# sleepybishop/nanorq

Measured on AMD Instinct MI355X. Metric: Gbit/s encode+decode, K=8192 T=1280, higher is better.
Workload: dtype u8

## Files before the change

__graft_entry__.py:

```python
import os
import sys

ROOT = os.path.dirname(os.path.abspath(__file__))
for p in (ROOT, os.path.join(ROOT, "tests")):
    if p not in sys.path:
        sys.path.insert(0, p)


def build():
    from nanorq_amd import build as nbuild
    nbuild.build_lib(verbose=True)
    nbuild.build_emu()
    nbuild.build_planner_emu()
    nbuild.build_ingest_emu()
    nbuild.build_emit_emu()
    nbuild.build_held_emu()
    nbuild.build_rxset_emu()
    nbuild.build_rxset_lists_emu()
    nbuild.build_txset_emu()
    nbuild.build_obj_emu()
    nbuild.build_shape_emu()
    nbuild.build_tools()
    import oracle
    oracle.build()
    if os.path.isfile("/root/reference/benchmark.c"):
        import subprocess
        subprocess.run(["make", "-s", "-C", os.path.join(ROOT, "oracle"), "_ref/benchmark_hip", "_ref/encode_hip", "_ref/decode_hip"],
                       check=True)
    import nanorq_amd
    nanorq_amd.lib()
    print("build ok:", nanorq_amd.lib_path())


def smoke():
    import numpy as np
# ... 29 lines not shown
```

nanorq_amd/binding.py:

```python
import ctypes as C
import os

import numpy as np

_HERE = os.path.dirname(os.path.abspath(__file__))
_LIB = None


class NrqError(RuntimeError):
    pass


class ObjParams(C.Structure):
    _fields_ = [("F", C.c_uint64)] + [(n, C.c_uint32) for n in
                                       ("T", "Al", "Z", "N", "Kt", "ZL", "KL", "KpL", "ZS", "KS", "KpS", "NL", "TL", "NS", "TS",
                                        "flags", "max_esi")] + [("oti_common", C.c_uint64), ("oti_specific", C.c_uint32)]

    def as_dict(self):
        return {n: getattr(self, n) for n, _ in self._fields_}


class CallStats(C.Structure):
    _fields_ = [("plan_ms", C.c_double), ("host_ms", C.c_double), ("strip_bytes", C.c_uint32),
                ("lds_bytes", C.c_uint32), ("grid", C.c_uint32), ("planner", C.c_uint32),
# ... 121 lines not shown
        L.nrq_rxset_decode.argtypes = [vp, ip, u32p]
    if hasattr(L, "nrq_txset_create"):
        L.nrq_txset_create.argtypes = [vp, C.c_uint32, C.POINTER(vp)]
        L.nrq_txset_destroy.argtypes = [vp]
        L.nrq_txset_destroy.restype = None
        L.nrq_txset_attach.argtypes = [vp, C.c_uint32, vp]
        L.nrq_txset_attach_obj.argtypes = [vp, C.c_uint32, vp]
        L.nrq_txset_detach.argtypes = [vp, C.c_uint32]
        L.nrq_txset_blocks.argtypes = [vp, u32p, u32p, C.c_uint32, u32p]
        L.nrq_txset_emit.argtypes = [vp, vp, vp, C.c_uint32, vp, sz, C.c_uint32, vp]
    u8pp = C.POINTER(C.POINTER(C.c_uint8))
    L.nrq_host_kconst_build.argtypes = [C.c_uint32, u8pp, u32p]
    L.nrq_host_plan_build.argtypes = [C.c_uint32, C.c_uint32, u32p, C.POINTER(C.c_uint8), u8pp, u32p]
    L.nrq_host_free.argtypes = [vp]
    L.nrq_host_free.restype = None
    _LIB = L
    return L


PARAM_NAMES = ("Kp", "J", "S", "H", "W", "L", "P", "P1", "U", "B")
PLAN_FIELDS = ("magic status K Kp J S H W L P P1 B M npiv u nlow r2 nfree nlev nrows pipe wpr "
               "npiv_pad n_xor_ops off_ops off_pivslot off_pivcol off_wt off_lowslot off_pivx off_fbits "
               "off_mh off_freex off_hinv off_colslot off_pivof off_uslot total_bytes reserved0 reserved1 fail_site "
               "off_augt lpr aug_stride nneed need_pad off_needslot off_wneed").split()


def params(K):
    out = (C.c_uint32 * 10)()
    if lib().nrq_params(K, out) != 0:
        raise ValueError("K out of range: %r" % (K,))
    return dict(zip(PARAM_NAMES, (int(x) for x in out)))


def _u32(a):
    return a.ctypes.data_as(C.POINTER(C.c_uint32))


def host_kconst(K):
    out = C.POINTER(C.c_uint8)()
    n = C.c_uint32()
    if lib().nrq_host_kconst_build(K, C.byref(out), C.byref(n)) != 0:
        raise NrqError("kconst build failed")
    buf = bytes(C.string_at(out, n.value))
    lib().nrq_host_free(out)
    return buf


# ... 664 lines not shown
```

nanorq_amd/build.py:

```python
import os
import shutil
import subprocess
import sys

HERE = os.path.dirname(os.path.abspath(__file__))
ROOT = os.path.dirname(HERE)
CSRC = os.path.join(HERE, "csrc")
LIB = os.path.join(HERE, "libnanorq_hip.so")
EMU = os.path.join(ROOT, "tests", "emu", "libsolve_emu.so")
PEMU = os.path.join(ROOT, "tests", "emu", "libplanner_emu.so")
IEMU = os.path.join(ROOT, "tests", "emu", "libingest_emu.so")
XEMU = os.path.join(ROOT, "tests", "emu", "libemit_emu.so")
OEMU = os.path.join(ROOT, "tests", "emu", "libobj_emu.so")
SEMU = os.path.join(ROOT, "tests", "emu", "libshape_emu.so")
HEMU = os.path.join(ROOT, "tests", "emu", "libheld_emu.so")
WEMU = os.path.join(ROOT, "tests", "emu", "libwant_emu.so")
REMU = os.path.join(ROOT, "tests", "emu", "librxset_emu.so")
LEMU = os.path.join(ROOT, "tests", "emu", "librxset_lists_emu.so")
TEMU = os.path.join(ROOT, "tests", "emu", "libtxset_emu.so")

HIP_SOURCES = ["nrq_device.hip"]
CXX_SOURCES = ["planner_host.cpp"]
C_SOURCES = ["nanorq_api.c", "io.c"]


def _hipcc():
    for c in (os.environ.get("HIPCC"), "/opt/rocm/bin/hipcc", shutil.which("hipcc")):
        if c and os.path.exists(c):
            return c
    raise RuntimeError("hipcc not found: the HIP extension cannot be built (no CPU fallback exists)")


def _newer(target, deps):
# ... 54 lines not shown
    return target


def build_tools(force=False):
    src = os.path.join(ROOT, "tools", "rqfile.c")
    exe = os.path.join(ROOT, "tools", "rqfile")
    deps = [src, LIB] + [os.path.join(ROOT, "include", h) for h in ("nanorq.h", "nanorq_batch.h", "io.h")]
    if force or _newer(exe, deps):
        subprocess.run(["gcc", "-std=c99", "-D_DEFAULT_SOURCE", "-D_FILE_OFFSET_BITS=64", "-O2", "-Wall", "-I" + os.path.join(ROOT, "include"),
                        src, "-o", exe, "-L" + os.path.dirname(LIB), "-lnanorq_hip", "-Wl,-rpath,$ORIGIN/../nanorq_amd", "-lm"], check=True)
    return exe


def _build_emu(target, src, headers, force):
    if force or _newer(target, [src] + [os.path.join(CSRC, h) for h in headers]):
        subprocess.run(["g++", "-O2", "-std=c++17", "-Wall", "-Wno-unknown-pragmas", "-fPIC", "-shared", "-o", target, src], check=True)
    return target


def build_emu(force=False):
    return _build_emu(EMU, os.path.join(ROOT, "tests", "emu", "solve_emu.cpp"), ("solve_body.h", "plan.h"), force)


def build_planner_emu(force=False):
    return _build_emu(PEMU, os.path.join(ROOT, "tests", "emu", "planner_emu.cpp"),
                      ("planner_body.h", "planner_seq.h", "solve_body.h", "plan.h", "rq_math.h"), force)


def build_ingest_emu(force=False):
    return _build_emu(IEMU, os.path.join(ROOT, "tests", "emu", "ingest_emu.cpp"), ("ingest_body.h",), force)


def build_emit_emu(force=False):
    return _build_emu(XEMU, os.path.join(CSRC, "emit_emu.cpp"), ("emit_body.h", "rq_math.h"), force)


def build_held_emu(force=False):
    return _build_emu(HEMU, os.path.join(CSRC, "held_emu.cpp"), ("emit_body.h", "held_body.h", "ingest_body.h", "rq_math.h"), force)


def build_want_emu(force=False):
    return _build_emu(WEMU, os.path.join(CSRC, "want_emu.cpp"), ("want_body.h", "held_body.h", "ingest_body.h"), force)


def build_rxset_emu(force=False):
    return _build_emu(REMU, os.path.join(CSRC, "rxset_emu.cpp"), ("ingest_set_body.h", "ingest_body.h"), force)


def build_rxset_lists_emu(force=False):
    return _build_emu(LEMU, os.path.join(CSRC, "rxset_lists_emu.cpp"),
                      ("lists_set_body.h", "rxset_plan.h", "ingest_set_body.h", "ingest_body.h"), force)


def build_txset_emu(force=False):
    return _build_emu(TEMU, os.path.join(CSRC, "txset_emu.cpp"), ("emit_set_body.h", "emit_body.h", "rq_math.h"), force)


def build_obj_emu(force=False):
    return _build_emu(OEMU, os.path.join(ROOT, "tests", "emu", "obj_emu.cpp"), ("obj_body.h", "emit_body.h", "rq_math.h"), force)


def build_shape_emu(force=False):
    return _build_emu(SEMU, os.path.join(ROOT, "tests", "emu", "shape_emu.cpp"),
                      ("launch_shape.h", "planner_body.h", "solve_body.h", "plan.h", "rq_math.h", "rfc6330_tables.h"), force)


if __name__ == "__main__":
    build_lib(force="-f" in sys.argv, verbose=True)
    build_emu(force="-f" in sys.argv)
    build_planner_emu(force="-f" in sys.argv)
    build_ingest_emu(force="-f" in sys.argv)
    build_emit_emu(force="-f" in sys.argv)
    build_held_emu(force="-f" in sys.argv)
    build_want_emu(force="-f" in sys.argv)
    build_rxset_emu(force="-f" in sys.argv)
    build_rxset_lists_emu(force="-f" in sys.argv)
    build_txset_emu(force="-f" in sys.argv)
    build_obj_emu(force="-f" in sys.argv)
    build_shape_emu(force="-f" in sys.argv)
    build_tools(force="-f" in sys.argv)
```

nanorq_amd/csrc/launch_shape.h:

```cpp
#ifndef NRQ_LAUNCH_SHAPE_H
#define NRQ_LAUNCH_SHAPE_H

#include <stdint.h>
#include <stdlib.h>
#include <string.h>

#include <vector>

#include "plan.h"
#include "rq_math.h"
#include "solve_body.h"
#include "planner_body.h"

#define NRQ_LDS_MAX 163840u
#define NRQ_LDS_GRANULE 1280u
static inline uint32_t lds_alloc(uint32_t bytes) { return (bytes + NRQ_LDS_GRANULE - 1u) / NRQ_LDS_GRANULE * NRQ_LDS_GRANULE; }
#ifndef NRQ_WG
#define NRQ_WG 768
#endif
#ifndef NRQ_TINY_WV
#define NRQ_TINY_WV 3
#endif
#ifndef NRQ_TINY_OCC
#define NRQ_TINY_OCC 12u
#endif
#ifndef NRQ_SMALL_WV
#define NRQ_SMALL_WV 4
#endif

static inline bool nrq_map_by_block(uint32_t nblk) { return nblk >= 64u || (nblk >= 8u && (nblk & 7u) == 0u); }

enum KnobKind { KNOB_FLAG, KNOB_NFLAG, KNOB_NUM, KNOB_BOOLNUM, KNOB_WIDEG, KNOB_LDSMAX };
#define NRQ_KNOBS(K)                                                                                                                                    \
  K(bool, map_spread, false, "NRQ_MAP_SPREAD", "map_spread", KNOB_FLAG)               \
  K(bool, big_wg, false, "NRQ_BIG_WG", "big_wg", KNOB_FLAG)                                                \
                                                                                                                          \
  K(bool, small_waves4, true, "NRQ_SMALL_WAVES5", "small_waves4", KNOB_NFLAG)                                                                           \
  K(bool, prof, false, "NRQ_PROF", 0, KNOB_FLAG)                                                   \
  K(bool, diag, false, "NRQ_DIAG", 0, KNOB_FLAG)                                                 \
  K(bool, plan_lds_max, false, "NRQ_PLAN_LDS_MAX", 0, KNOB_FLAG)                                                \
  K(bool, plan_big_wg, false, "NRQ_PLAN_BIG_WG", "plan_big_wg", KNOB_FLAG)                                             \
  K(uint32_t, small_div, 2, "NRQ_SMALL_DIV", 0, KNOB_NUM)        \
  K(uint64_t, solve_grid, 0, "NRQ_SOLVE_GRID", "solve_grid", KNOB_NUM)             \
  K(uint32_t, max_wb, 16, "NRQ_MAX_WB", "max_wb", KNOB_NUM)                                                                \
  K(bool, no_wb12, false, "NRQ_NO_WB12", "no_wb12", KNOB_FLAG)                                       \
                                                                                                    \
  K(bool, tiny_any, false, "NRQ_TINY_ANY", "tiny_any", KNOB_FLAG)                                                                                       \
  K(bool, plan_pack, false, "NRQ_PLAN_PACK", "plan_pack", KNOB_FLAG)          \
                                                              \
  K(bool, host_plan_auto, true, "NRQ_HOST_PLAN_AUTO", "host_plan_auto", KNOB_BOOLNUM)                                                                   \
  K(int, prof_base, 2, "NRQ_PROF_BASE", 0, KNOB_NUM)                                    \
                                                                                                        \
  K(uint32_t, encplan_dev_min_l, 12000, "NRQ_ENCPLAN_DEV_MIN_L", "encplan_dev_min_l", KNOB_NUM)                                                         \
  K(uint32_t, wide_g, 0, "NRQ_WIDE_G", "wide_g", KNOB_WIDEG)           \
                                                                  \
  K(bool, no_wentry, false, "NRQ_NO_WENTRY", "no_wentry", KNOB_FLAG)                                                                                    \
  K(bool, no_tiny, false, "NRQ_NO_TINY", "no_tiny", KNOB_FLAG)                                     \
                                                                                                            \
  K(uint32_t, tiny_div, 7, "NRQ_TINY_DIV", "tiny_div", KNOB_NUM)                                                                                        \
                                                                                                             \
  K(uint32_t, tiny_div_dec, 7, "NRQ_TINY_DIV_DEC", "tiny_div_dec", KNOB_NUM)                                                                            \
  K(bool, no_split, false, "NRQ_NO_SPLIT", "no_split", KNOB_FLAG)                \
  K(bool, no_balance, false, "NRQ_NO_BALANCE", "no_balance", KNOB_FLAG)            \
                                                    \
  K(uint32_t, lds_max, NRQ_LDS_MAX, 0, "lds_max", KNOB_LDSMAX)                                                                                          \
                                                                \
  K(bool, no_lists, false, "NRQ_NO_LISTS", "no_lists", KNOB_FLAG)                                                                                       \
  K(int, reserve_cus, -1, "NRQ_RESERVE_CUS", "reserve_cus", KNOB_NUM)  \
// ... 332 lines not shown
```

nanorq_amd/csrc/nrq_device.hip:

```cpp
#include <hip/hip_runtime.h>

#include <algorithm>
#include <atomic>
#include <chrono>
#include <cstdarg>
#include <cstdio>
#include <cstdlib>
#include <cstring>
#include <deque>
#include <map>
#include <new>
#include <string>
#include <thread>
#include <vector>

#include "../../include/nanorq_hip.h"
#include "plan.h"
#include "planner_host.h"
#include "rq_math.h"
#include "solve_body.h"
#include "planner_body.h"
#include "ingest_body.h"
#include "ingest_set_body.h"
#include "lists_set_body.h"
// ... 52 lines not shown
#endif
#ifndef NRQ_BIG_RING
#define NRQ_BIG_RING NRQ_RING_MAX
#endif
#ifndef NRQ_PROF_DONE
#define NRQ_PROF_DONE 9
#endif
#ifndef NRQ_W12_FW
#define NRQ_W12_FW 3
#endif
#ifndef NRQ_W12_GW
#define NRQ_W12_GW 2
#endif
#ifndef NRQ_W12_SW
#define NRQ_W12_SW 2
#endif
template <int WB, int NT, int WV, int G = 1, bool AL = false>
__global__ __launch_bounds__(NT) __attribute__((amdgpu_waves_per_eu(WV)))
void nrq_solve_kernel(const nrq_job *__restrict__ jobs, uint32_t nblk,
                                                       uint32_t T, uint32_t nstrips, uint32_t by_block, uint32_t nslots,
                                                       uint32_t lsub, const uint8_t *__restrict__ kc,
                                                       uint8_t *__restrict__ stage_all, uint32_t stage_stride,
                                                       uint32_t ostage_stride, unsigned long long *__restrict__ prof,
                                                       uint8_t *__restrict__ ybuf, size_t ybuf_stride) {
  extern __shared__ __attribute__((aligned(16))) uint8_t smem[];
  const uint32_t tid = threadIdx.x;
  static_assert(G == 1 || WB == 16, "wide strips are made of 16-byte lanes");
  static_assert(WB != 12 || NT >= 512, "12-byte strips: the 768-thread workgroup only (blocks whose 16-byte image does not fit the LDS)");
  constexpr uint32_t WBE = (uint32_t)WB * G;
  constexpr bool ALX = AL && G == 1 && WB >= 4;
  const uint32_t vt = tid / G, subl = tid % G;
  constexpr uint32_t VNT = NT / G;
  constexpr uint32_t SPL = nrq_group_strips(WBE), NFW = (G == 1 && WB == 12 && NT >= 512) ? (uint32_t)NRQ_W12_FW : (G == 1 && WB >= 8 && NT >= 512) ? 2u : 1u,
                     NMV = (NT / 64u) / 4u * (4u - NFW) + ((NT / 64u) % 4u > NFW ? (NT / 64u) % 4u - NFW : 0u),
                     NGW = NFW == 3u ? (uint32_t)NRQ_W12_GW : NMV >= 6u ? (WB <= NRQ_GATHER_WAVES_NARROW_WB ? NRQ_GATHER_WAVES_NARROW : NRQ_MOVER_WAVES) : NMV >= 3u ? 2u : 1u,
                     NSW = NFW == 3u ? (uint32_t)NRQ_W12_SW : NMV >= 6u ? NRQ_MOVER_WAVES : NMV - NGW;
  static_assert(NMV >= 2u || NT == 64, "workgroup too small for the data movers");
#ifndef NRQ_PIPE_SMALL
#define NRQ_PIPE_SMALL 0
#endif
#ifndef NRQ_PIPE_BIG
#define NRQ_PIPE_BIG 1
#endif
  constexpr bool MPIPE = (NRQ_PIPE_BIG && NT >= 512) || (NRQ_PIPE_SMALL && NT == 256 && WV == 4);
#ifndef NRQ_RING_4W
#define NRQ_RING_4W NRQ_RING
#endif
// ... 195 lines not shown
        ph_combine<WB, G>(c, w0, vt, VNT, cb_);
        __syncthreads();
      }
      if (lpr_) {
        ph_clear_x<WB, G>(c, vt, VNT);
        __syncthreads();
      }
      NRQ_STAMP(4);
      NRQ_STOP(3)
#ifndef NRQ_FOLD_PRE256
#define NRQ_FOLD_PRE256 0
#endif
      ph_dense_fold<WB, G, (NT == 64 ? 8 : NT == 256 ? NRQ_FOLD_PRE256 : 0)>(c, vt, VNT);
      __syncthreads();
      NRQ_MARK(c, 4);
      if (dense_fold_shared(VNT) || G > 1) {
        ph_hdpc_reduce<WB, G>(c, vt, VNT);
        __syncthreads();
      }
      NRQ_MARK(c, 5);
      ph_dense_free<WB, G, (NT == 64)>(c, vt, VNT);
      __syncthreads();
      NRQ_MARK(c, 6);
      ph_dense_cu<WB, G, (NT == 64)>(c, vt, VNT);
      __syncthreads();
      NRQ_STAMP(5);
      NRQ_STOP(4)
      if (ybuf) {
        NRQ_STAMP(6);
        NRQ_STAMP(7);
        ph_store_raw<WB, G>(c, ostage_cur + (size_t)sidx * ostage_stride + subl * WB, vt, VNT);
      } else {
        ph_tables<WB, G>(c, vt, VNT);
        __syncthreads();
        NRQ_STAMP(6);
        NRQ_STOP(5)
        ph_backsub<WB, G, (NT >= 512)>(c, vt, VNT);
        ph_park<WB, G>(c, vt, VNT);
        __syncthreads();
        NRQ_STAMP(7);
        NRQ_STOP(6)
        ph_store<WB, G, (NT >= 512)>(c, ostage_cur + (size_t)sidx * ostage_stride + subl * WB, vt, VNT);
      }
      __syncthreads();
      NRQ_STAMP(8);
#undef NRQ_STAMP
#undef NRQ_STOP
    }
    __syncthreads();
    qp = q;
    q = qn;
    buf ^= 1u;
  }
  if (qp < nslots) {
    GroupDst<WB> gp;
    const uint32_t units_p = group_dst(qp, gp) << lsub;
    pf_scatter_impl<WB, G, MPIPE, ALX>(gp, ostage0 + (size_t)(buf ^ 1u) * SPL * ostage_stride, ostage_stride, 0u, units_p, (tid) / G, (NT) / G, subl);
  }
}

enum {
// ... 880 lines not shown
    rc = 1;
    if (ctx->planner && p.L >= ctx->tune.encplan_dev_min_l) rc = encplan_device_launch(ctx, p, K, kc, ep);
    if (rc < 0) return rc;
    if (rc > 0) return encplan_host_build(ctx, p, K, kc, ep);
  }
  return finish ? encplan_finish(ctx, p, K, kc, ep) : 0;
}

void build_out_lists(const rq_params &p, const uint16_t *colslot, uint32_t n, const uint32_t *isis,
                     std::vector<uint32_t> &cptr, std::vector<uint16_t> &cols) {
  cptr.resize(n + 1);
  cols.clear();
  cols.reserve((size_t)n * 9);
  uint32_t tmp[RQ_MAX_LT_COLS];
  for (uint32_t q = 0; q < n; q++) {
    cptr[q] = (uint32_t)cols.size();
    uint32_t m = rq_lt_columns(&p, isis[q], tmp);
    for (uint32_t k = 0; k < m; k++) cols.push_back(colslot[tmp[k]]);
  }
  cptr[n] = (uint32_t)cols.size();
}

using solve_fn = void (*)(const nrq_job *, uint32_t, uint32_t, uint32_t, uint32_t, uint32_t, uint32_t, const uint8_t *, uint8_t *, uint32_t,
                          uint32_t, unsigned long long *, uint8_t *, size_t);
#define NRQ_SOLVE_ROW(WB, NT, WV, G, AL) &nrq_solve_kernel<WB, NT, WV, G, AL>,
static const solve_fn solve_table[] = {NRQ_SOLVE_INSTANCES(NRQ_SOLVE_ROW)};
#undef NRQ_SOLVE_ROW

static int launch_solve(nrq_ctx *ctx, const std::vector<const nrq_plan_hdr *> &hdrs, const nrq_job *d_jobs, uint32_t nblk,
                        uint32_t T, const uint8_t *d_kc, uint32_t max_out, uint32_t wb, uint32_t need, bool io_aligned) {
  SolveIn in;
  in.wb = wb; in.nblk = nblk; in.T = T; in.lds_bytes = need; in.max_out = max_out; in.io_aligned = io_aligned;
  in.hdrs = hdrs.data(); in.nhdrs = hdrs.size();
  for (const nrq_plan_hdr *h : hdrs) {
    if (h->status) continue;
    if (h->M > in.max_slots) in.max_slots = h->M;
    if (h->u > in.max_u) in.max_u = h->u;
    if (h->wpr > in.max_wpr) in.max_wpr = h->wpr;
  }
  const SolveShape s = solve_shape(ctx->tune, ctx->ncu, ctx->ahead_hint, in);
  if (s.err == SHAPE_GRID_TOO_LARGE) return fail(ctx, -4, "grid too large");
  if (s.key.NT == 64 && ctx->tune.diag) fprintf(stderr, "[NRQ_DIAG] single-wave workgroups: %u bytes of LDS each, %u per CU\n", s.lds_bytes, s.occ);
  const int inst = solve_key_index(s.key);
  if (inst < 0)
    return fail(ctx, -2, "no solve kernel instance <%d, %d, %d, %d, %s>", s.key.WB, s.key.NT, s.key.WV, s.key.G, s.key.AL ? "true" : "false");
  {
    int rc_ = ensure_dev(ctx, ctx->stage, s.stage_bytes());
// ... 10 lines not shown
                                    hipFuncAttributeMaxDynamicSharedMemorySize, (int)NRQ_LDS_MAX));
    HIPCHK(ctx, hipFuncSetAttribute(reinterpret_cast<const void *>(&nrq_backsub_kernel<16>),
                                    hipFuncAttributeMaxDynamicSharedMemorySize, (int)NRQ_LDS_MAX));
    for (int i = 0; i < nrq_solve_nkeys; i++)
      if (nrq_solve_keys[i].WB == (int)wb)
        HIPCHK(ctx, hipFuncSetAttribute(reinterpret_cast<const void *>(solve_table[i]), hipFuncAttributeMaxDynamicSharedMemorySize,
                                        (int)NRQ_LDS_MAX));
    ctx->attr_widths |= 1u << wb;
  }
  hipEvent_t ev1 = nullptr;
  if (ctx->ktime_on && !ctx->ktime_outer) {
    int rc_ = timing_pair(ctx, ctx->ktime_pool, ctx->ktime_used, ctx->stream, &ev1);
    if (rc_) return rc_;
  }
  const uint32_t nprof = (s.grid + 15u) / 16u;
  DevBuf prof;
  if (ctx->tune.prof) {
    HIPCHK(ctx, hipMalloc((void **)&prof.p, (size_t)nprof * 16 * 8));
    HIPCHK(ctx, hipMemsetAsync(prof.p, 0, (size_t)nprof * 16 * 8, ctx->stream));
  }
  unsigned long long *const d_prof = reinterpret_cast<unsigned long long *>(prof.p);
  hipLaunchKernelGGL(solve_table[inst], dim3(s.grid), dim3((uint32_t)s.key.NT), s.lds_bytes, ctx->stream, d_jobs, nblk, T, s.nstrips,
                     s.by_block ? 1u : 0u, s.nslots, s.lsub, d_kc, (uint8_t *)ctx->stage.p, s.stage_stride, s.ostage_stride, d_prof, ybuf,
                     s.ybuf_stride);
  if (s.key.G == 1) ctx->stats.movers_aligned = s.key.AL ? 1u : 0u;
  HIPCHK(ctx, hipGetLastError());
  if (s.split) {
    if (s.err == SHAPE_BACKSUB_TABLES) return fail(ctx, -5, "back-substitution tables do not fit the LDS (wpr=%u)", in.max_wpr);
    const dim3 bgrid(s.backsub_nsb, s.nchunks, nblk);
    if (s.backsub_strip == 32u)
      hipLaunchKernelGGL(nrq_backsub_kernel<32>, bgrid, dim3(256), s.backsub_tbl, ctx->stream, d_jobs, T, ybuf, s.ybuf_stride, s.nchunks);
    else
      hipLaunchKernelGGL(nrq_backsub_kernel<16>, bgrid, dim3(256), s.backsub_tbl, ctx->stream, d_jobs, T, ybuf, s.ybuf_stride, s.nchunks);
    HIPCHK(ctx, hipGetLastError());
    if (s.res_elems) {
      hipLaunchKernelGGL(nrq_collect_kernel, dim3(s.res_elems, nblk), dim3(256), 0, ctx->stream, d_jobs, T, (const uint8_t *)ybuf, s.ybuf_stride);
      HIPCHK(ctx, hipGetLastError());
    }
  }
  if (ev1) HIPCHK(ctx, hipEventRecord(ev1, ctx->stream));
  if (d_prof) {
    std::vector<unsigned long long> hp((size_t)nprof * 16);
    HIPCHK(ctx, hipMemcpyAsync(hp.data(), d_prof, hp.size() * 8, hipMemcpyDeviceToHost, ctx->stream));
    HIPCHK(ctx, hipStreamSynchronize(ctx->stream));
    static const char *names[8] = {"load", "fwd", "hdpc", "bin", "dense", "tables", "backsub", "store"};
    double sum[8] = {0}, tot = 0;
    uint32_t cnt = 0;
// ... 3619 lines not shown
```

nanorq_amd/csrc/plan.h:

```cpp
#ifndef NRQ_PLAN_H
#define NRQ_PLAN_H

#include <stdint.h>

#define NRQ_PLAN_MAGIC 0x4e525131u
#define NRQ_ROW 64u
#ifndef NRQ_PIPE
#define NRQ_PIPE 2u
#endif
#ifndef NRQ_RING_MULT
#define NRQ_RING_MULT 5u
#endif
#define NRQ_RING (NRQ_RING_MULT * 4u * (NRQ_PIPE + 1u))
#define NRQ_RING_MAX (2u * NRQ_RING)
#define NRQ_PAD_ROWS (2u * NRQ_RING_MAX + NRQ_PIPE + 4u)
#define NRQ_OP_INDEX(row, lane) ((((size_t)(row) >> 2) * NRQ_ROW + (size_t)(lane)) * 4u + ((size_t)(row) & 3u))
#define NRQ_OP_LANE_OF_INDEX(i) ((uint32_t)((i) >> 2) & (NRQ_ROW - 1u))
#define NRQ_STREAM_ROWS(rows) (((rows) + 3u) & ~3u)
#define NRQ_SCRATCH 64u
#define NRQ_OP(dst, src) (((uint32_t)(dst) + NRQ_SCRATCH) | (((uint32_t)(src) + NRQ_SCRATCH) << 16))
#define NRQ_NOP_AT(pos) (((uint32_t)(pos) & (NRQ_ROW - 1u)) * 0x10001u)
#define NRQ_OP_IS_NOP(op) (((op) & 0xFFFFu) < NRQ_SCRATCH)
#define NRQ_OP_DST(op) (((op) & 0xFFFFu) - NRQ_SCRATCH)
#define NRQ_OP_SRC(op) (((op) >> 16) - NRQ_SCRATCH)
#define NRQ_NOSLOT 0xFFFFu
#define NRQ_MAX_FREE 32u

#define NRQ_LANE_CLASSES 8u
// ... 53 lines not shown
  uint32_t off_ops;
  uint32_t off_pivslot;
  uint32_t off_pivcol;
  uint32_t off_wt;
  uint32_t off_lowslot;
  uint32_t off_pivx;
  uint32_t off_fbits;
  uint32_t off_mh;
  uint32_t off_freex;
  uint32_t off_hinv;
  uint32_t off_colslot;
  uint32_t off_pivof;
  uint32_t off_uslot;
  uint32_t total_bytes;
  uint32_t reserved[2];
  uint32_t fail_site;
  uint32_t off_augt;
  uint32_t lpr;
  uint32_t aug_stride;
  uint32_t nneed;
  uint32_t need_pad;
  uint32_t off_needslot;
  uint32_t off_wneed;
} nrq_plan_hdr;
#ifdef __cplusplus
static_assert(sizeof(nrq_plan_hdr) <= 256u, "nrq_plan_hdr is read as a 256-byte prefix");
#endif

#define NRQ_CHEAD 16u
typedef struct nrq_kconst_hdr {
  uint32_t Kp, S, H, n;
  uint32_t off_g;
  uint32_t off_b12;
  uint32_t total_bytes;
  uint32_t L, W, P, nnz;
  uint32_t off_rptr;
  uint32_t off_cidx;
  uint32_t off_cptr;
  uint32_t off_ridx;
  uint32_t off_state;
  uint32_t off_gt;
  uint32_t off_erow;
  uint32_t off_chead;
} nrq_kconst_hdr;

#endif
// ... 1 lines not shown
```

nanorq_amd/csrc/planner_host.cpp:

```cpp
#include <algorithm>
#include <cstdlib>
#include <cstring>
#include <vector>

#include "plan.h"
#include "planner_host.h"
#include "rq_math.h"

namespace {

struct GF {
  uint8_t exp[510], log[256], inv[256];
  GF() {
    uint32_t x = 1;
    for (int e = 0; e < 255; e++) {
      exp[e] = (uint8_t)x;
      log[x] = (uint8_t)e;
      x <<= 1;
      if (x & 0x100) x ^= 0x11D;
    }
    for (int e = 255; e < 510; e++) exp[e] = exp[e - 255];
    log[0] = 0; inv[0] = 0;
    for (int v = 1; v < 256; v++) inv[v] = exp[255 - log[v]];
  }
// ... 545 lines not shown
        for (uint32_t w = 0; w < aw; w++) aug[(size_t)h * aw + w] ^= gf.mul(b, aug[(size_t)pr * aw + w]);
      }
    }
    if (!status)
      for (uint32_t f = 0; f < nfree; f++)
        for (uint32_t h = 0; h < H; h++) hinv[(size_t)f * H + h] = aug[(size_t)solver[f] * aw + nfree + h];
  }

  std::vector<uint16_t> colslot(L, NRQ_NOSLOT), pivof(n_hd, NRQ_NOSLOT), uslot(u, NRQ_NOSLOT);
  for (uint32_t k = 0; k < npiv; k++) {
    colslot[pivcol[k]] = pivslot[k];
    pivof[pivcol[k]] = pivslot[k];
  }
  {
    uint32_t x = 0;
    for (uint32_t r = 0; r < M && x < u; r++)
      if (!assigned[r]) { uslot[x] = (uint16_t)r; colslot[ucol[x]] = (uint16_t)r; x++; }
    if (x != u) return -5;
  }

  Arena A;
  nrq_plan_hdr hd;
  memset(&hd, 0, sizeof(hd));
  A.buf.reserve(ops.size() * 4u + (size_t)wpr * ((npiv + 63u) & ~63u) * 4u + (size_t)L * 16u + (size_t)augt.size() * 4u + 8192u);
  A.reserve((uint32_t)sizeof(hd));
  hd.magic = NRQ_PLAN_MAGIC; hd.status = status;
  hd.K = K; hd.Kp = p.Kp; hd.J = p.J; hd.S = S; hd.H = H; hd.W = W; hd.L = L; hd.P = p.P; hd.P1 = p.P1; hd.B = p.B;
  hd.M = M; hd.npiv = npiv; hd.u = u; hd.nlow = nlow; hd.r2 = r2; hd.nfree = nfree; hd.nlev = nlev;
  hd.nrows = op_rows; hd.pipe = NRQ_PIPE; hd.wpr = wpr;
  hd.npiv_pad = (npiv + 63u) & ~63u;
  hd.n_xor_ops = n_real_ops;
  {
    while ((ops.size() / NRQ_ROW) % 4u) pad_rows(1);
    hd.off_ops = A.reserve((uint32_t)(ops.size() * 4));
    uint32_t *out = A.at<uint32_t>(hd.off_ops);
    const size_t nquads = ops.size() / (4u * NRQ_ROW);
    for (size_t g = 0; g < nquads; g++) {
      const uint32_t *r0 = &ops[g * 4u * NRQ_ROW];
      uint32_t *o = out + g * 4u * NRQ_ROW;
      for (uint32_t l = 0; l < NRQ_ROW; l++) {
        o[4u * l] = r0[l]; o[4u * l + 1u] = r0[NRQ_ROW + l]; o[4u * l + 2u] = r0[2u * NRQ_ROW + l]; o[4u * l + 3u] = r0[3u * NRQ_ROW + l];
      }
    }
  }
  hd.off_pivslot = A.reserve(npiv * 2);
  memcpy(A.at<uint8_t>(hd.off_pivslot), pivslot.data(), (size_t)npiv * 2);
  hd.off_pivcol = A.reserve(npiv * 2);
// ... 5 lines not shown
      for (uint32_t w = 0; w < wpr; w++) wt[(size_t)w * hd.npiv_pad + k] = Wm[(size_t)k * wpr + w];
  }
  hd.off_lowslot = A.reserve(std::max(1u, nlow) * 2);
  if (nlow) memcpy(A.at<uint8_t>(hd.off_lowslot), lowslot.data(), (size_t)nlow * 2);
  hd.off_pivx = A.reserve(std::max(1u, r2) * 2);
  for (uint32_t q = 0; q < r2; q++) A.at<uint16_t>(hd.off_pivx)[q] = (uint16_t)red_x[q];
  hd.off_fbits = A.reserve(std::max(1u, r2) * 4);
  memcpy(A.at<uint8_t>(hd.off_fbits), fbits.data(), (size_t)std::max(1u, r2) * 4);
  hd.off_mh = A.reserve(H * std::max(1u, r2));
  memcpy(A.at<uint8_t>(hd.off_mh), mh.data(), (size_t)H * std::max(1u, r2));
  hd.off_freex = A.reserve(std::max(1u, nfree) * 2);
  for (uint32_t f = 0; f < nfree; f++) A.at<uint16_t>(hd.off_freex)[f] = (uint16_t)freex[f];
  hd.off_hinv = A.reserve(std::max(1u, nfree) * H);
  memcpy(A.at<uint8_t>(hd.off_hinv), hinv.data(), (size_t)std::max(1u, nfree) * H);
  hd.off_colslot = A.reserve(L * 2);
  memcpy(A.at<uint8_t>(hd.off_colslot), colslot.data(), (size_t)L * 2);
  hd.off_pivof = A.reserve(n_hd * 2);
  memcpy(A.at<uint8_t>(hd.off_pivof), pivof.data(), (size_t)n_hd * 2);
  hd.off_uslot = A.reserve(std::max(1u, u) * 2);
  if (u) memcpy(A.at<uint8_t>(hd.off_uslot), uslot.data(), (size_t)u * 2);
  hd.lpr = aug_in_stream ? 0u : lpr; hd.aug_stride = aug_stride;
  hd.off_augt = A.reserve((uint32_t)(augt.size() * 4 + 16));
  if (!augt.empty()) memcpy(A.at<uint8_t>(hd.off_augt), augt.data(), augt.size() * 4);
  hd.total_bytes = align16((uint32_t)A.buf.size());
  A.buf.resize(hd.total_bytes, 0);
  memcpy(A.buf.data(), &hd, sizeof(hd));

  uint8_t *res = (uint8_t *)malloc(hd.total_bytes);
  if (!res) return -2;
  memcpy(res, A.buf.data(), hd.total_bytes);
  *out = res;
  *out_bytes = hd.total_bytes;
  return 0;
}

extern "C" int nrq_host_plan_build(uint32_t K, uint32_t nrows, const uint32_t *isis, const uint8_t *kconst, uint8_t **out, uint32_t *out_bytes) {
  rq_params p;
  if (!rq_params_init(K, &p)) return -1;
  bool encoder = nrows == p.Kp;
  for (uint32_t k = 0; encoder && k < nrows; k++) encoder = isis[k] == k;
  uint32_t way = !encoder ? 0u : p.Kp >= 1500u ? 1u : 6u;
  if (const char *e = getenv("NRQ_HOST_WAY")) { if (encoder) way = (uint32_t)atoi(e); }
  return host_plan_build_with(K, nrows, isis, kconst, out, out_bytes, way);
}
```

nanorq_amd/csrc/solve_body.h:

```cpp
#ifndef NRQ_SOLVE_BODY_H
#define NRQ_SOLVE_BODY_H

#include <stdint.h>
#include <string.h>

#include "plan.h"

#if defined(__HIPCC__)
#define SB_HD __host__ __device__ __forceinline__
#define SB_MEM __host__ __device__ __forceinline__
#else
#define SB_HD static inline
#define SB_MEM inline
struct uint2 { uint32_t x, y; };
struct uint4 { uint32_t x, y, z, w; };
#endif

#if defined(__HIP_DEVICE_COMPILE__)
#define NRQ_GAS __attribute__((address_space(1)))
#else
#define NRQ_GAS
#endif
template <class X> SB_HD const NRQ_GAS X *gptr(const void *p) { return (const NRQ_GAS X *)p; }
template <class X> SB_HD const NRQ_GAS X *gptr(uint64_t p) { return (const NRQ_GAS X *)(uintptr_t)p; }
// ... 365 lines not shown
  nrq_lds_layout l;
  uint32_t o = 0;
  o = NRQ_SCRATCH * WB;
  l.off_slots = o; o = nrq_r16(o + (h->M + h->r2) * WB);
  l.off_cu = o;    o = nrq_r16(o + (h->u ? h->u : 1u) * WB);
  uint32_t cf = NRQ_MAX_FREE * WB;
  uint32_t t4 = h->wpr * 8u * 16u * (WB == 12u ? 16u : WB);
  l.off_x = o;
  o = nrq_r16(o + (cf > t4 ? cf : t4));
  l.total = o;
  return l;
}

template <int WB, int G = 1> struct StripCtx {
  const uint8_t *plan;
  const nrq_plan_hdr *h;
  const uint8_t *kc;
  const nrq_job *job;
  uint8_t *lds;
  nrq_lds_layout lay;
  uint32_t T, strip, valid;
  unsigned long long *dbg = nullptr;
  bool dbg_t0 = false;
  SB_MEM uint8_t *slots() const { return lds + lay.off_slots; }
  SB_MEM uint8_t *cu() const { return lds + lay.off_cu; }
  SB_MEM uint8_t *cf() const { return lds + lay.off_x; }
  SB_MEM uint8_t *t4() const { return lds + lay.off_x; }
  template <class X> SB_MEM const NRQ_GAS X *arr(uint32_t off) const { return gptr<X>(plan + off); }
};

template <int WB> struct GroupSrc {
  const NRQ_GAS uint32_t *rowsrc;
  const NRQ_GAS uint8_t *src, *rep;
  uint32_t M, T, strip0, nstrips;
  uint32_t lsub;
};
template <int WB, int CB> SB_HD SV<WB> chunk_piece(const SV<CB> &v, int j) {
  SV<WB> r = sv_zero<WB>();
  if constexpr (WB == 8) { r.w[0] = v.w[2 * j]; r.w[1] = v.w[2 * j + 1]; }
  else if constexpr (WB == 4) r.w[0] = v.w[j];
  else r.w[0] = (v.w[j >> 1] >> ((j & 1) * 16)) & 0xFFFFu;
  return r;
}
template <int WB, int CB, bool PIPELINED> SB_HD void pf_gather_chunks(const GroupSrc<WB> &g, NRQ_GAS uint8_t *stage, size_t stage_stride, uint32_t u0,
                                                                      uint32_t u1, uint32_t p, uint32_t np) {
#ifndef NRQ_GATHER_CHUNK_PB
// ... 828 lines not shown
    uint4 t; t.x = v.w[0]; t.y = v.w[1]; t.z = v.w[2]; t.w = 0u;
    reinterpret_cast<uint4 *>(t4)[e] = t;
  } else lds_put<WB, G>(t4, e, v);
}
template <int WB, int G = 1> SB_HD void ph_tables(const StripCtx<WB, G> &c, uint32_t tid, uint32_t nt) {
  const uint32_t ngroups = c.h->wpr * 8u, u = c.h->u;
  for (uint32_t e = tid; e < ngroups * 16u; e += nt) {
    uint32_t grp = e >> 4, nib = e & 15u;
    SV<WB> v = sv_zero<WB>();
#pragma unroll
    for (uint32_t bq = 0; bq < 4; bq++) {
      uint32_t x = grp * 4u + bq;
      if (((nib >> bq) & 1u) && x < u) {
        SV<WB> t = lds_get<WB, G>(c.cu(), x);
        sv_xor<WB>(v, t);
      }
    }
    t4_put<WB, G>(c.t4(), e, v);
  }
}

template <int WB, int NW, int G = 1, bool FAST = true>
SB_HD void backsub_one(const StripCtx<WB, G> &c, const uint8_t *t4, uint32_t slot, const uint32_t (&bitsw)[NW],
                       uint32_t wpr) {
  SV<WB> acc = lds_get<WB, G>(c.slots(), slot);
#pragma unroll
  for (uint32_t w = 0; w < (uint32_t)NW; w++) {
    if (w >= wpr) break;
    const uint32_t bits = bitsw[w];
#if defined(__HIP_DEVICE_COMPILE__)
    if constexpr (WB == 16 && G == 1) {
      uint32_t odd = bits & 0xF0F0F0F0u, even = (bits << 4) & 0xF0F0F0F0u;
      asm volatile("" : "+v"(odd), "+v"(even));
      if constexpr (FAST) {
      const uint32_t tbw = (uint32_t)(uintptr_t)t4 + w * 2048u;
      uint4 d[8];
#pragma unroll
      for (uint32_t q = 0; q < 8; q++) d[q] = *NRQ_LDSP(uint4, t4_addr(tbw, (q & 1u) ? odd : even, q >> 1) + q * 256u);
#pragma unroll
      for (uint32_t q = 0; q < 8; q += 2) {
        acc.w[0] = nrq_xor3(acc.w[0], d[q].x, d[q + 1].x); acc.w[1] = nrq_xor3(acc.w[1], d[q].y, d[q + 1].y);
        acc.w[2] = nrq_xor3(acc.w[2], d[q].z, d[q + 1].z); acc.w[3] = nrq_xor3(acc.w[3], d[q].w, d[q + 1].w);
      }
      } else {
        const uint32_t tb = (uint32_t)(uintptr_t)t4;
#pragma unroll
      for (uint32_t q = 0; q < 8; q++) {
// ... 28 lines not shown
#pragma unroll
      for (uint32_t q = 0; q < 8; q++) d[q] = *NRQ_LDSP(uint4, t4_addr(tbw, (q & 1u) ? odd : even, q >> 1) + q * 256u);
      uint32_t pad = 0;
#pragma unroll
      for (uint32_t q = 0; q < 8; q += 2) {
        acc.w[0] = nrq_xor3(acc.w[0], d[q].x, d[q + 1].x); acc.w[1] = nrq_xor3(acc.w[1], d[q].y, d[q + 1].y);
        acc.w[2] = nrq_xor3(acc.w[2], d[q].z, d[q + 1].z); pad = nrq_xor3(pad, d[q].w, d[q + 1].w);
      }
      asm volatile("" : : "v"(pad));
      NRQ_SCHED_FENCE();
      continue;
    }
#endif
#pragma unroll
    for (uint32_t q = 0; q < 8; q++) {
      const uint32_t nib = (bits >> (4u * q)) & 15u;
      SV<WB> t = t4_get<WB, G>(t4, (w * 8u + q) * 16u + nib);
      sv_xor<WB>(acc, t);
      if (q == 3) NRQ_SCHED_FENCE();
    }
    NRQ_SCHED_FENCE();
  }
  lds_put<WB, G>(c.slots(), slot, acc);
}

#define NRQ_BACKSUB_VIEW(c, need)                                                                                            \
  const NRQ_GAS uint16_t *pivslot = (c).template arr<uint16_t>((need) ? (c).h->off_needslot : (c).h->off_pivslot);      \
  const NRQ_GAS uint32_t *wt = (c).template arr<uint32_t>((need) ? (c).h->off_wneed : (c).h->off_wt);                   \
  const uint32_t stride = (need) ? (c).h->need_pad : (c).h->npiv_pad, npiv = (need) ? (c).h->nneed : (c).h->npiv
template <int WB, int NW, int G = 1, bool FAST = true>
SB_HD void backsub_fixed(const StripCtx<WB, G> &c, bool need, uint32_t tid, uint32_t nt) {
  if constexpr (!FAST) {

  NRQ_BACKSUB_VIEW(c, need);
  const uint32_t wpr = c.h->wpr;
  const uint8_t *t4 = c.t4();
  for (uint32_t k = tid; k < npiv; k += 2 * nt) {
    const uint32_t k2 = k + nt;
    uint32_t a[NW], b[NW];
    const uint32_t sa = pivslot[k];
    const uint32_t sb = k2 < npiv ? pivslot[k2] : 0u;
#pragma unroll
    for (uint32_t w = 0; w < (uint32_t)NW; w++) a[w] = w < wpr ? wt[(size_t)w * stride + k] : 0u;
#pragma unroll
    for (uint32_t w = 0; w < (uint32_t)NW; w++) b[w] = (w < wpr && k2 < npiv) ? wt[(size_t)w * stride + k2] : 0u;
    backsub_one<WB, NW, G, false>(c, t4, sa, a, wpr);
    if (k2 < npiv) backsub_one<WB, NW, G, false>(c, t4, sb, b, wpr);
  }
    return;
  }
  NRQ_BACKSUB_VIEW(c, need);
  const uint32_t wpr = c.h->wpr;
  const uint8_t *t4 = c.t4();
  uint32_t a[NW], b[NW], sa = 0, sb = 0;
  uint32_t k = tid;
  if (k < npiv) {
    sa = pivslot[k];
#pragma unroll
    for (uint32_t w = 0; w < (uint32_t)NW; w++) a[w] = w < wpr ? wt[(size_t)w * stride + k] : 0u;
  }
  for (; k < npiv; k += 2 * nt) {
    const uint32_t k2 = k + nt, k3 = k + 2 * nt;
    if (k2 < npiv) {
      sb = pivslot[k2];
#pragma unroll
      for (uint32_t w = 0; w < (uint32_t)NW; w++) b[w] = w < wpr ? wt[(size_t)w * stride + k2] : 0u;
    }
    backsub_one<WB, NW, G, FAST>(c, t4, sa, a, wpr);
    if (k3 < npiv) {
      sa = pivslot[k3];
#pragma unroll
      for (uint32_t w = 0; w < (uint32_t)NW; w++) a[w] = w < wpr ? wt[(size_t)w * stride + k3] : 0u;
    }
    if (k2 < npiv) backsub_one<WB, NW, G, FAST>(c, t4, sb, b, wpr);
  }
}

template <int WB, int G = 1, bool FAST = true> SB_HD void ph_backsub(const StripCtx<WB, G> &c, uint32_t tid, uint32_t nt) {
  const uint32_t wpr = c.h->wpr;
  const bool need = c.job->inter == 0 && c.h->off_needslot != 0u;
  if (wpr <= 4) backsub_fixed<WB, 4, G, FAST>(c, need, tid, nt);
  else if (wpr <= 8) backsub_fixed<WB, 8, G, FAST>(c, need, tid, nt);
  else if (wpr <= 12) backsub_fixed<WB, 12, G, FAST>(c, need, tid, nt);
  else if (wpr <= 24) backsub_fixed<WB, 24, G, FAST>(c, need, tid, nt);
  else {
    NRQ_BACKSUB_VIEW(c, need);
    const uint8_t *t4 = c.t4();
    for (uint32_t k = tid; k < npiv; k += nt) {
      uint32_t s = pivslot[k];
      SV<WB> acc = lds_get<WB, G>(c.slots(), s);
      for (uint32_t w = 0; w < wpr; w++) {
        uint32_t bits = wt[(size_t)w * stride + k];
#pragma unroll
        for (uint32_t q = 0; q < 8; q++) {
          uint32_t nib = (bits >> (4u * q)) & 15u;
          SV<WB> t = t4_get<WB, G>(t4, (w * 8u + q) * 16u + nib);
          sv_xor<WB>(acc, t);
        }
      }
      lds_put<WB, G>(c.slots(), s, acc);
    }
  }
}

template <int WB, int G = 1> SB_HD void ph_park(const StripCtx<WB, G> &c, uint32_t tid, uint32_t nt) {
  const NRQ_GAS uint16_t *uslot = c.template arr<uint16_t>(c.h->off_uslot);
  for (uint32_t x = tid; x < c.h->u; x += nt) lds_put<WB, G>(c.slots(), uslot[x], lds_get<WB, G>(c.cu(), x));
}

#ifndef NRQ_STORE_CHUNK
#define NRQ_STORE_CHUNK 8u
#endif
#ifndef NRQ_STORE_TRIP
#define NRQ_STORE_TRIP 32u
#endif
#define NRQ_STORE_SLACK (16u + NRQ_STORE_TRIP * 4u)
#define NRQ_LT_LIST_MAX 33u
static_assert(NRQ_LT_LIST_MAX <= 2u * NRQ_STORE_TRIP, "ph_store reads at most two trips of a list; out_slots[] slack is sized for that");
template <int WB, int G = 1> SB_HD uint32_t out_elems(const nrq_job *job, const nrq_plan_hdr *h) { return (job->inter ? h->L : 0u) + job->nout; }
SB_HD void store_trip(const NRQ_GAS uint16_t *osl, uint32_t e, uint32_t end, uint32_t (&raw)[NRQ_STORE_TRIP / 2u]) {
  (void)end;
#ifdef __HIP_DEVICE_COMPILE__
  typedef uint32_t u4 __attribute__((ext_vector_type(4)));
  typedef u4 u4a __attribute__((aligned(2)));
#pragma unroll
  for (uint32_t k = 0; k < NRQ_STORE_TRIP / 8u; k++) {
    const u4 w = *reinterpret_cast<const NRQ_GAS u4a *>(osl + e + 8u * k);
    raw[4u * k] = w.x; raw[4u * k + 1u] = w.y; raw[4u * k + 2u] = w.z; raw[4u * k + 3u] = w.w;
  }
#else
#pragma unroll
  for (uint32_t k = 0; k < NRQ_STORE_TRIP / 2u; k++)
    raw[k] = (e + 2u * k < end ? (uint32_t)osl[e + 2u * k] : 0u) | (e + 2u * k + 1u < end ? (uint32_t)osl[e + 2u * k + 1u] : 0u) << 16;
#endif
}
SB_HD uint32_t store_slot(const uint32_t (&raw)[NRQ_STORE_TRIP / 2u], uint32_t k, uint32_t e, uint32_t end, uint32_t zero_at) {
  return e + k < end ? ((raw[k / 2u] >> (16u * (k & 1u))) & 0xFFFFu) + NRQ_SCRATCH : zero_at;
}
template <int WB, int G = 1, bool FAST = true> SB_HD void ph_store(const StripCtx<WB, G> &c, NRQ_GAS uint8_t *ostage, uint32_t tid, uint32_t nt) {
  constexpr int STB = 8;
  const NRQ_GAS uint16_t *colslot = c.template arr<uint16_t>(c.h->off_colslot);
  const uint32_t L = c.h->L, ni = c.job->inter ? L : 0u;
  for (uint32_t base = tid; base < ni; base += STB * nt) {
    uint32_t sl[STB];
#pragma unroll
    for (int q = 0; q < STB; q++) {
      uint32_t col = base + (uint32_t)q * nt;
      sl[q] = col < L ? colslot[col] : 0u;
    }
#pragma unroll
    for (int q = 0; q < STB; q++) {
      uint32_t col = base + (uint32_t)q * nt;
      if (col < L) g_put_stream<WB>(ostage + (size_t)col * (WB * G), WB, lds_get<WB, G>(c.slots(), sl[q]));
    }
  }
  const NRQ_GAS uint32_t *cptr = gptr<uint32_t>(c.job->out_cptr);
  const NRQ_GAS uint16_t *osl = gptr<uint16_t>(c.job->out_slots);
  if constexpr (FAST) {
  const uint32_t nout = c.job->nout;
  constexpr uint32_t CH = NRQ_STORE_CHUNK;
  const uint32_t zero_at = tid & (NRQ_SCRATCH - 1u);
  uint32_t e_n = 0, end_n = 0;
  if (tid < nout) { e_n = cptr[tid]; end_n = cptr[tid + 1]; }
  const uint32_t npass = (nout + nt - 1u) / nt;
  for (uint32_t pass = 0, q = tid; pass < npass; pass++, q += nt) {
    uint32_t e = e_n;
// ... 169 lines not shown
```

Before: 1627.

## Fuse intermediate-symbol store into back-substitution via column-ordered weight table

Adds a column-indexed copy of the back-substitution weight matrix to the plan so back-substitution can iterate over all L columns and stream each finished intermediate symbol straight to the output stage. The separate LDS-to-global copy loop in ph_store is then skipped, and park runs before backsub. This removes one pass over LDS slots and a separate store phase when intermediates are requested. In exchange the plan grows by wpr*L words, backsub does more rows (L instead of npiv, non-pivot columns with zero weights), and the plan magic changes.

Measured after the change: 1631 (median of 6 runs). Within noise of the previous version (+0.3%).

```diff
diff --git a/__graft_entry__.py b/__graft_entry__.py
--- a/__graft_entry__.py
+++ b/__graft_entry__.py
@@ -11,6 +11,7 @@
     from nanorq_amd import build as nbuild
     nbuild.build_lib(verbose=True)
     nbuild.build_emu()
+    nbuild.build_fused_store_emu()
     nbuild.build_planner_emu()
     nbuild.build_ingest_emu()
     nbuild.build_emit_emu()
diff --git a/nanorq_amd/binding.py b/nanorq_amd/binding.py
--- a/nanorq_amd/binding.py
+++ b/nanorq_amd/binding.py
@@ -167,7 +167,8 @@
 PLAN_FIELDS = ("magic status K Kp J S H W L P P1 B M npiv u nlow r2 nfree nlev nrows pipe wpr "
                "npiv_pad n_xor_ops off_ops off_pivslot off_pivcol off_wt off_lowslot off_pivx off_fbits "
                "off_mh off_freex off_hinv off_colslot off_pivof off_uslot total_bytes reserved0 reserved1 fail_site "
-               "off_augt lpr aug_stride nneed need_pad off_needslot off_wneed").split()
+               "off_augt lpr aug_stride nneed need_pad off_needslot off_wneed "
+               "off_wcol col_pad").split()
 
 
 def params(K):
diff --git a/nanorq_amd/build.py b/nanorq_amd/build.py
--- a/nanorq_amd/build.py
+++ b/nanorq_amd/build.py
@@ -9,6 +9,7 @@
 LIB = os.path.join(HERE, "libnanorq_hip.so")
 EMU = os.path.join(ROOT, "tests", "emu", "libsolve_emu.so")
 PEMU = os.path.join(ROOT, "tests", "emu", "libplanner_emu.so")
+FEMU = os.path.join(ROOT, "tests", "emu", "libfused_store_emu.so")
 IEMU = os.path.join(ROOT, "tests", "emu", "libingest_emu.so")
 XEMU = os.path.join(ROOT, "tests", "emu", "libemit_emu.so")
 OEMU = os.path.join(ROOT, "tests", "emu", "libobj_emu.so")
@@ -109,6 +110,10 @@
     return _build_emu(EMU, os.path.join(ROOT, "tests", "emu", "solve_emu.cpp"), ("solve_body.h", "plan.h"), force)
 
 
+def build_fused_store_emu(force=False):
+    return _build_emu(FEMU, os.path.join(ROOT, "tests", "emu", "fused_store_emu.cpp"), ("solve_body.h", "plan.h"), force)
+
+
 def build_planner_emu(force=False):
     return _build_emu(PEMU, os.path.join(ROOT, "tests", "emu", "planner_emu.cpp"),
                       ("planner_body.h", "planner_seq.h", "solve_body.h", "plan.h", "rq_math.h"), force)
@@ -155,6 +160,7 @@
 if __name__ == "__main__":
     build_lib(force="-f" in sys.argv, verbose=True)
     build_emu(force="-f" in sys.argv)
+    build_fused_store_emu(force="-f" in sys.argv)
     build_planner_emu(force="-f" in sys.argv)
     build_ingest_emu(force="-f" in sys.argv)
     build_emit_emu(force="-f" in sys.argv)
diff --git a/nanorq_amd/csrc/launch_shape.h b/nanorq_amd/csrc/launch_shape.h
--- a/nanorq_amd/csrc/launch_shape.h
+++ b/nanorq_amd/csrc/launch_shape.h
@@ -44,6 +44,8 @@
   K(uint64_t, solve_grid, 0, "NRQ_SOLVE_GRID", "solve_grid", KNOB_NUM)             \
   K(uint32_t, max_wb, 16, "NRQ_MAX_WB", "max_wb", KNOB_NUM)                                                                \
   K(bool, no_wb12, false, "NRQ_NO_WB12", "no_wb12", KNOB_FLAG)                                       \
+                        \
+  K(bool, no_fused_tail, false, "NRQ_NO_FUSED_TAIL", "no_fused_tail", KNOB_FLAG)                                                                        \
                                                                                                     \
   K(bool, tiny_any, false, "NRQ_TINY_ANY", "tiny_any", KNOB_FLAG)                                                                                       \
   K(bool, plan_pack, false, "NRQ_PLAN_PACK", "plan_pack", KNOB_FLAG)          \
diff --git a/nanorq_amd/csrc/nrq_device.hip b/nanorq_amd/csrc/nrq_device.hip
--- a/nanorq_amd/csrc/nrq_device.hip
+++ b/nanorq_amd/csrc/nrq_device.hip
@@ -98,7 +98,7 @@
                                                        uint32_t lsub, const uint8_t *__restrict__ kc,
                                                        uint8_t *__restrict__ stage_all, uint32_t stage_stride,
                                                        uint32_t ostage_stride, unsigned long long *__restrict__ prof,
-                                                       uint8_t *__restrict__ ybuf, size_t ybuf_stride) {
+                                                       uint8_t *__restrict__ ybuf, size_t ybuf_stride, uint32_t no_fused_tail) {
   extern __shared__ __attribute__((aligned(16))) uint8_t smem[];
   const uint32_t tid = threadIdx.x;
   static_assert(G == 1 || WB == 16, "wide strips are made of 16-byte lanes");
@@ -340,6 +340,9 @@
       ph_dense_free<WB, G, (NT == 64)>(c, vt, VNT);
       __syncthreads();
       NRQ_MARK(c, 6);
+      if constexpr (NT >= 512 && G == 1 && (WB == 16 || WB == 12 || WB == 8)) {
+        if (!ybuf && !no_fused_tail) offer_fused_tail<WB, G>(c, ostage_cur + (size_t)sidx * ostage_stride);
+      }
       ph_dense_cu<WB, G, (NT == 64)>(c, vt, VNT);
       __syncthreads();
       NRQ_STAMP(5);
@@ -349,12 +352,14 @@
         NRQ_STAMP(7);
         ph_store_raw<WB, G>(c, ostage_cur + (size_t)sidx * ostage_stride + subl * WB, vt, VNT);
       } else {
+        const bool fused = fused_tail<WB, G, (NT >= 512)>(c);
+        if (fused) ph_park<WB, G>(c, vt, VNT);
         ph_tables<WB, G>(c, vt, VNT);
         __syncthreads();
         NRQ_STAMP(6);
         NRQ_STOP(5)
         ph_backsub<WB, G, (NT >= 512)>(c, vt, VNT);
-        ph_park<WB, G>(c, vt, VNT);
+        if (!fused) ph_park<WB, G>(c, vt, VNT);
         __syncthreads();
         NRQ_STAMP(7);
         NRQ_STOP(6)
@@ -1281,7 +1286,7 @@
 }
 
 using solve_fn = void (*)(const nrq_job *, uint32_t, uint32_t, uint32_t, uint32_t, uint32_t, uint32_t, const uint8_t *, uint8_t *, uint32_t,
-                          uint32_t, unsigned long long *, uint8_t *, size_t);
+                          uint32_t, unsigned long long *, uint8_t *, size_t, uint32_t);
 #define NRQ_SOLVE_ROW(WB, NT, WV, G, AL) &nrq_solve_kernel<WB, NT, WV, G, AL>,
 static const solve_fn solve_table[] = {NRQ_SOLVE_INSTANCES(NRQ_SOLVE_ROW)};
 #undef NRQ_SOLVE_ROW
@@ -1338,7 +1343,7 @@
   unsigned long long *const d_prof = reinterpret_cast<unsigned long long *>(prof.p);
   hipLaunchKernelGGL(solve_table[inst], dim3(s.grid), dim3((uint32_t)s.key.NT), s.lds_bytes, ctx->stream, d_jobs, nblk, T, s.nstrips,
                      s.by_block ? 1u : 0u, s.nslots, s.lsub, d_kc, (uint8_t *)ctx->stage.p, s.stage_stride, s.ostage_stride, d_prof, ybuf,
-                     s.ybuf_stride);
+                     s.ybuf_stride, ctx->tune.no_fused_tail ? 1u : 0u);
   if (s.key.G == 1) ctx->stats.movers_aligned = s.key.AL ? 1u : 0u;
   HIPCHK(ctx, hipGetLastError());
   if (s.split) {
diff --git a/nanorq_amd/csrc/plan.h b/nanorq_amd/csrc/plan.h
--- a/nanorq_amd/csrc/plan.h
+++ b/nanorq_amd/csrc/plan.h
@@ -3,7 +3,7 @@
 
 #include <stdint.h>
 
-#define NRQ_PLAN_MAGIC 0x4e525131u
+#define NRQ_PLAN_MAGIC 0x4e525132u
 #define NRQ_ROW 64u
 #ifndef NRQ_PIPE
 #define NRQ_PIPE 2u
@@ -103,6 +103,8 @@
   uint32_t need_pad;
   uint32_t off_needslot;
   uint32_t off_wneed;
+  uint32_t off_wcol;
+  uint32_t col_pad;
 } nrq_plan_hdr;
 #ifdef __cplusplus
 static_assert(sizeof(nrq_plan_hdr) <= 256u, "nrq_plan_hdr is read as a 256-byte prefix");
diff --git a/nanorq_amd/csrc/planner_host.cpp b/nanorq_amd/csrc/planner_host.cpp
--- a/nanorq_amd/csrc/planner_host.cpp
+++ b/nanorq_amd/csrc/planner_host.cpp
@@ -591,7 +591,8 @@
   Arena A;
   nrq_plan_hdr hd;
   memset(&hd, 0, sizeof(hd));
-  A.buf.reserve(ops.size() * 4u + (size_t)wpr * ((npiv + 63u) & ~63u) * 4u + (size_t)L * 16u + (size_t)augt.size() * 4u + 8192u);
+  A.buf.reserve(ops.size() * 4u + (size_t)wpr * (((npiv + 63u) & ~63u) + ((L + 63u) & ~63u)) * 4u + (size_t)L * 16u + (size_t)augt.size() * 4u +
+                8192u);
   A.reserve((uint32_t)sizeof(hd));
   hd.magic = NRQ_PLAN_MAGIC; hd.status = status;
   hd.K = K; hd.Kp = p.Kp; hd.J = p.J; hd.S = S; hd.H = H; hd.W = W; hd.L = L; hd.P = p.P; hd.P1 = p.P1; hd.B = p.B;
@@ -643,6 +644,13 @@
   hd.lpr = aug_in_stream ? 0u : lpr; hd.aug_stride = aug_stride;
   hd.off_augt = A.reserve((uint32_t)(augt.size() * 4 + 16));
   if (!augt.empty()) memcpy(A.at<uint8_t>(hd.off_augt), augt.data(), augt.size() * 4);
+  hd.col_pad = (L + 63u) & ~63u;
+  hd.off_wcol = A.reserve(wpr * hd.col_pad * 4);
+  {
+    uint32_t *wcol = A.at<uint32_t>(hd.off_wcol);
+    for (uint32_t k = 0; k < npiv; k++)
+      for (uint32_t w = 0; w < wpr; w++) wcol[(size_t)w * hd.col_pad + pivcol[k]] = Wm[(size_t)k * wpr + w];
+  }
   hd.total_bytes = align16((uint32_t)A.buf.size());
   A.buf.resize(hd.total_bytes, 0);
   memcpy(A.buf.data(), &hd, sizeof(hd));
diff --git a/nanorq_amd/csrc/solve_body.h b/nanorq_amd/csrc/solve_body.h
--- a/nanorq_amd/csrc/solve_body.h
+++ b/nanorq_amd/csrc/solve_body.h
@@ -411,6 +411,7 @@
   uint32_t T, strip, valid;
   unsigned long long *dbg = nullptr;
   bool dbg_t0 = false;
+  NRQ_GAS uint8_t *ostage = nullptr;
   SB_MEM uint8_t *slots() const { return lds + lay.off_slots; }
   SB_MEM uint8_t *cu() const { return lds + lay.off_cu; }
   SB_MEM uint8_t *cf() const { return lds + lay.off_x; }
@@ -1285,7 +1286,7 @@
 
 template <int WB, int NW, int G = 1, bool FAST = true>
 SB_HD void backsub_one(const StripCtx<WB, G> &c, const uint8_t *t4, uint32_t slot, const uint32_t (&bitsw)[NW],
-                       uint32_t wpr) {
+                       uint32_t wpr, NRQ_GAS uint8_t *ost = nullptr, uint32_t elem = 0u) {
   SV<WB> acc = lds_get<WB, G>(c.slots(), slot);
 #pragma unroll
   for (uint32_t w = 0; w < (uint32_t)NW; w++) {
@@ -1360,17 +1361,29 @@
     NRQ_SCHED_FENCE();
   }
   lds_put<WB, G>(c.slots(), slot, acc);
-}
-
-#define NRQ_BACKSUB_VIEW(c, need)                                                                                            \
-  const NRQ_GAS uint16_t *pivslot = (c).template arr<uint16_t>((need) ? (c).h->off_needslot : (c).h->off_pivslot);      \
-  const NRQ_GAS uint32_t *wt = (c).template arr<uint32_t>((need) ? (c).h->off_wneed : (c).h->off_wt);                   \
-  const uint32_t stride = (need) ? (c).h->need_pad : (c).h->npiv_pad, npiv = (need) ? (c).h->nneed : (c).h->npiv
+  if (ost) g_put_stream<WB>(ost + (size_t)elem * (WB * G), WB, acc);
+}
+
+template <int WB, int G = 1> SB_HD void offer_fused_tail(StripCtx<WB, G> &c, NRQ_GAS uint8_t *ostage) {
+  c.ostage = (c.job->inter != 0 && c.h->off_wcol != 0u) ? ostage : nullptr;
+}
+template <int WB, int G = 1, bool FAST = true> SB_HD bool fused_tail(const StripCtx<WB, G> &c) {
+  if constexpr (FAST && G == 1 && (WB == 16 || WB == 12 || WB == 8)) return c.ostage != nullptr;
+  else return false;
+}
+
+#define NRQ_BACKSUB_VIEW(c, need, col)                                                                                                          \
+  const NRQ_GAS uint16_t *pivslot = (c).template arr<uint16_t>((col) ? (c).h->off_colslot : (need) ? (c).h->off_needslot : (c).h->off_pivslot); \
+  const NRQ_GAS uint32_t *wt = (c).template arr<uint32_t>((col) ? (c).h->off_wcol : (need) ? (c).h->off_wneed : (c).h->off_wt);                 \
+  const uint32_t stride = (col) ? (c).h->col_pad : (need) ? (c).h->need_pad : (c).h->npiv_pad,                                                  \
+                 npiv = (col) ? (c).h->L : (need) ? (c).h->nneed : (c).h->npiv;                                                                 \
+  NRQ_GAS uint8_t *const ost = (col) ? (c).ostage : nullptr
 template <int WB, int NW, int G = 1, bool FAST = true>
-SB_HD void backsub_fixed(const StripCtx<WB, G> &c, bool need, uint32_t tid, uint32_t nt) {
+SB_HD void backsub_fixed(const StripCtx<WB, G> &c, bool need, bool col, uint32_t tid, uint32_t nt) {
   if constexpr (!FAST) {
 
-  NRQ_BACKSUB_VIEW(c, need);
+  NRQ_BACKSUB_VIEW(c, need, false);
+  (void)ost; (void)col;
   const uint32_t wpr = c.h->wpr;
   const uint8_t *t4 = c.t4();
   for (uint32_t k = tid; k < npiv; k += 2 * nt) {
@@ -1387,7 +1400,7 @@
   }
     return;
   }
-  NRQ_BACKSUB_VIEW(c, need);
+  NRQ_BACKSUB_VIEW(c, need, col);
   const uint32_t wpr = c.h->wpr;
   const uint8_t *t4 = c.t4();
   uint32_t a[NW], b[NW], sa = 0, sb = 0;
@@ -1404,25 +1417,26 @@
 #pragma unroll
       for (uint32_t w = 0; w < (uint32_t)NW; w++) b[w] = w < wpr ? wt[(size_t)w * stride + k2] : 0u;
     }
-    backsub_one<WB, NW, G, FAST>(c, t4, sa, a, wpr);
+    backsub_one<WB, NW, G, FAST>(c, t4, sa, a, wpr, ost, k);
     if (k3 < npiv) {
       sa = pivslot[k3];
 #pragma unroll
       for (uint32_t w = 0; w < (uint32_t)NW; w++) a[w] = w < wpr ? wt[(size_t)w * stride + k3] : 0u;
     }
-    if (k2 < npiv) backsub_one<WB, NW, G, FAST>(c, t4, sb, b, wpr);
+    if (k2 < npiv) backsub_one<WB, NW, G, FAST>(c, t4, sb, b, wpr, ost, k2);
   }
 }
 
 template <int WB, int G = 1, bool FAST = true> SB_HD void ph_backsub(const StripCtx<WB, G> &c, uint32_t tid, uint32_t nt) {
   const uint32_t wpr = c.h->wpr;
   const bool need = c.job->inter == 0 && c.h->off_needslot != 0u;
-  if (wpr <= 4) backsub_fixed<WB, 4, G, FAST>(c, need, tid, nt);
-  else if (wpr <= 8) backsub_fixed<WB, 8, G, FAST>(c, need, tid, nt);
-  else if (wpr <= 12) backsub_fixed<WB, 12, G, FAST>(c, need, tid, nt);
-  else if (wpr <= 24) backsub_fixed<WB, 24, G, FAST>(c, need, tid, nt);
+  const bool col = fused_tail<WB, G, FAST>(c);
+  if (wpr <= 4) backsub_fixed<WB, 4, G, FAST>(c, need, col, tid, nt);
+  else if (wpr <= 8) backsub_fixed<WB, 8, G, FAST>(c, need, col, tid, nt);
+  else if (wpr <= 12) backsub_fixed<WB, 12, G, FAST>(c, need, col, tid, nt);
+  else if (wpr <= 24) backsub_fixed<WB, 24, G, FAST>(c, need, col, tid, nt);
   else {
-    NRQ_BACKSUB_VIEW(c, need);
+    NRQ_BACKSUB_VIEW(c, need, col);
     const uint8_t *t4 = c.t4();
     for (uint32_t k = tid; k < npiv; k += nt) {
       uint32_t s = pivslot[k];
@@ -1437,6 +1451,7 @@
         }
       }
       lds_put<WB, G>(c.slots(), s, acc);
+      if (ost) g_put_stream<WB>(ost + (size_t)k * (WB * G), WB, acc);
     }
   }
 }
@@ -1479,7 +1494,8 @@
   constexpr int STB = 8;
   const NRQ_GAS uint16_t *colslot = c.template arr<uint16_t>(c.h->off_colslot);
   const uint32_t L = c.h->L, ni = c.job->inter ? L : 0u;
-  for (uint32_t base = tid; base < ni; base += STB * nt) {
+  const uint32_t ncopy = fused_tail<WB, G, FAST>(c) ? 0u : ni;
+  for (uint32_t base = tid; base < ncopy; base += STB * nt) {
     uint32_t sl[STB];
 #pragma unroll
     for (int q = 0; q < STB; q++) {
```
